# nicklashansen/tdmpc2

Measured on AMD Instinct MI355X. Metric: plan() calls/sec (H=3, 512 samples, 6 iters), higher is better.
Workload: dtype f32 (f16x2-split products: 22-bit operands, fp32 accumulate)

## Files before the change

tdmpc2_amd/csrc/fused_kernels.cuh:

```cuda
#pragma once

#include "kloop_schedule.h"

#ifdef SPLIT_TIMING
#define TIMER_FIELDS mutable unsigned long long t_acc[14] = {0, 0, 0, 0, 0, 0, 0, 0, 0, 0, 0, 0, 0, 0}; mutable unsigned long long t_last = 0, t_begin = 0;
#define TIMER_START(c) { (c).t_last = (c).t_begin = __builtin_amdgcn_s_memtime(); }
#define TIMER_MARK(c, cls) { __builtin_amdgcn_sched_barrier(0); const unsigned long long t_now = __builtin_amdgcn_s_memtime(); __builtin_amdgcn_sched_barrier(0); (c).t_acc[cls] += t_now - (c).t_last; (c).t_last = t_now; }
#ifndef SPLIT_TIMING_WAVE
#define SPLIT_TIMING_WAVE 4
#endif
#define TIMER_FLUSH(c, ptr) if ((ptr) && threadIdx.x == 64 * SPLIT_TIMING_WAVE) { for (int i_ = 0; i_ < 14; ++i_) atomicAdd((ptr) + i_, (c).t_acc[i_]); atomicAdd((ptr) + 14, (c).t_last - (c).t_begin); atomicAdd((ptr) + 15, 1ull); }
#else
#define TIMER_FIELDS
#define TIMER_START(c)
#define TIMER_MARK(c, cls)
#define TIMER_FLUSH(c, ptr)
#endif
enum { T_KLOOP = 0, T_EPI = 1, T_HEAD = 2, T_ACT = 3, T_PARK = 4, T_TILE = 5, T_EPI_PRE = 6, T_EPI_SYNC = 7, T_EPI_BIAS = 8,
       T_EPI_COMB = 9, T_EPI_MATH = 10, T_CL_WAIT = 11, T_HEAD_K = 12, T_HEAD_ST = 13 };



#ifdef KS_NO_BIAS_LDS
constexpr bool KS_BIAS_LDS = false;
#else
constexpr bool KS_BIAS_LDS = true;
#endif
#ifdef KS_NO_ZH_REGS
constexpr bool KS_ZH_REGS = false;
#else
constexpr bool KS_ZH_REGS = true;
#endif
template <int APAD, int ST = 2, int NW = 8, int AR = 0>
struct CtxT {
    static constexpr bool BIAS_LDS = false;
    static constexpr int NST = ST;
    static constexpr int NWAVES = NW;
    static constexpr int ARITH = AR;
    static constexpr int FT = 16 / NW;
    static constexpr int NTHR = 64 * NW;
    static constexpr int TROWS = 32 * ST;
    static constexpr int SH = WIDTH + APAD;
    static constexpr int RSH = 2 * SH + 8;
    static constexpr int RSF_ = AR == 0 ? RSH / 2 : WIDTH + APAD + 4;
    static constexpr int KBLK = AR == 0 ? 16 : 8;
    static constexpr int ZKB = WIDTH / KBLK;
    _Float16 *act;
    float *stats;
    float *gb;
    int tid, wave, lane;
    mutable float pg[(WIDTH + NTHR - 1) / NTHR], pb[(WIDTH + NTHR - 1) / NTHR];
    TIMER_FIELDS
    __device__ __forceinline__ float *f32() const { return reinterpret_cast<float *>(act); }
    static constexpr __device__ __forceinline__ int RSF() { return RSF_; }
};
template <int APAD, int ST, int NW, int AR>
struct CtxPhT : CtxT<APAD, ST, NW, AR> {
    static constexpr bool BIAS_LDS = KS_BIAS_LDS;
    mutable float pbias = 0.f;
};

__device__ __forceinline__ float mish_fast(float x) {
    const float e = __expf(fminf(x, 20.f));
    const float n = e * (e + 2.f);
    return x * (n * __builtin_amdgcn_rcpf(n + 2.f));
}

template <class CT>
__device__ __forceinline__ float exp_a(float x) {
    if constexpr (CT::ARITH == 1) return expf(x);
    else return __expf(x);
}
template <class CT>
__device__ __forceinline__ float mish_a(float x) {
    if constexpr (CT::ARITH == 1) {
        const float e = expf(fminf(x, 20.f));
        const float n = e * (e + 2.f);
        return x * (n / (n + 2.f));
    } else {
        return mish_fast(x);
    }
}

__device__ __forceinline__ void split4(const f32x4 y, f16x4 &hi, f16x4 &lo, const float scale = ACT_SCALE) {
#pragma unroll
    for (int e = 0; e < 4; ++e) {
        const float ys = y[e] * scale;
        const _Float16 h = (_Float16)ys;
        hi[e] = h;
        lo[e] = (_Float16)(ys - (float)h);
    }
}


constexpr int PF = 2;
template <int FT>
struct BFragT {
    f16x8 h[FT], l[FT];
};
__device__ __forceinline__ f16x8 ldw(const char *ubase, unsigned voff, int imm) {
    return *reinterpret_cast<const f16x8 *>(ubase + voff + imm);
}
#define SPLIT_MFMA(a, b, c) __builtin_amdgcn_mfma_f32_32x32x16_f16(a, b, c, 0, 0, 0)
template <int FT>
__device__ __forceinline__ void load_b(BFragT<FT> &b, const char *u0, size_t ct_stride, unsigned voff) {
#pragma unroll
    for (int cc = 0; cc < FT; ++cc) {
        b.h[cc] = ldw(u0 + cc * ct_stride, voff, 0);
        b.l[cc] = ldw(u0 + cc * ct_stride, voff, 1024);
    }
}
template <int ST, int FT>
__device__ __forceinline__ void zero_acc(f32x16 (&a)[ST][FT]) {
#pragma unroll
    for (int r = 0; r < ST; ++r)
#pragma unroll
        for (int cc = 0; cc < FT; ++cc)
#pragma unroll
            for (int e = 0; e < 16; ++e) a[r][cc][e] = 0.f;
}
template <int ST>
struct AFragT {
    f16x8 h[ST], l[ST];
};
template <class CT>
__device__ __forceinline__ void load_a(AFragT<CT::NST> &a, const _Float16 *a0p, int kk) {
#pragma unroll
    for (int st = 0; st < CT::NST; ++st) {
        a.h[st] = *reinterpret_cast<const f16x8 *>(a0p + st * 32 * CT::RSH + kk * 16);
        a.l[st] = *reinterpret_cast<const f16x8 *>(a0p + st * 32 * CT::RSH + CT::SH + kk * 16);
    }
}
template <class CT>
__device__ __forceinline__ void kloop_f32(const CT &c, const LayerS &ly, int kb0, int kb1, f32x16 (&acc)[CT::NST][CT::FT]) {
    constexpr int FT = CT::FT, NST = CT::NST;
    constexpr int PFD = 4;
    const int i = c.lane & 31, hh = c.lane >> 5;
    const float *a0p = c.f32() + i * CT::RSF() + 4 * hh + kb0 * 8;
    const char *u0 = reinterpret_cast<const char *>(ly.wp) + ((size_t)(FT * c.wave) * ly.KB + kb0) * 1024;
    const size_t cts = (size_t)ly.KB * 1024;
    unsigned voff = (unsigned)c.lane * 16u;
    asm volatile("" : "+v"(voff));
    const int nk = kb1 - kb0;
    f32x4 ring[PFD][FT];
#pragma unroll
    for (int d = 0; d < PFD; ++d) {
        const int kd = d < nk ? d : nk - 1;
#pragma unroll
        for (int cc = 0; cc < FT; ++cc) ring[d][cc] = *reinterpret_cast<const f32x4 *>(u0 + (size_t)kd * 1024 + cc * cts + voff);
    }
    f32x4 an[NST];
#pragma unroll
    for (int st = 0; st < NST; ++st) an[st] = *reinterpret_cast<const f32x4 *>(a0p + st * 32 * CT::RSF());
    __builtin_amdgcn_sched_barrier(0);
#pragma unroll 1
    for (int k = 0; k < nk; k += PFD) {
#pragma unroll
        for (int d = 0; d < PFD; ++d) {
            const int kk = k + d;
            if (kk < nk) {
                f32x4 a[NST];
                const int kx = kk + 1 < nk ? kk + 1 : kk;
#pragma unroll
                for (int st = 0; st < NST; ++st) {
                    a[st] = an[st];
                    an[st] = *reinterpret_cast<const f32x4 *>(a0p + st * 32 * CT::RSF() + kx * 8);
                }
#pragma unroll
                for (int r = 0; r < 4; ++r)
#pragma unroll
                    for (int cc = 0; cc < FT; ++cc)
#pragma unroll
                        for (int st = 0; st < NST; ++st)
                            acc[st][cc] = __builtin_amdgcn_mfma_f32_32x32x2f32(ring[d][cc][r], a[st][r], acc[st][cc], 0, 0, 0);
                const int kn = kk + PFD < nk ? kk + PFD : nk - 1;
#pragma unroll
                for (int cc = 0; cc < FT; ++cc)
                    ring[d][cc] = *reinterpret_cast<const f32x4 *>(u0 + (size_t)kn * 1024 + cc * cts + voff);
                __builtin_amdgcn_sched_barrier(0);
            }
        }
    }
}

#define A_MFMA(ACC, WF, AF) asm volatile("v_mfma_f32_32x32x16_f16 %0, %1, %2, %0" : "+v"(ACC) : "v"(WF), "v"(AF))
template <int OFF>
__device__ __forceinline__ void a_dsrd(f16x8 &dst, unsigned addr) {
    asm volatile("ds_read_b128 %0, %1 offset:%2" : "=v"(dst) : "v"(addr), "n"(OFF));
}
__device__ __forceinline__ unsigned lds_addr_of(const void *p) {
    return (unsigned)(size_t)(const __attribute__((address_space(3))) char *)(p);
}
template <class CT>
__device__ __forceinline__ void a_load_act(AFragT<CT::NST> &a, unsigned la0, unsigned la1) {
    a_dsrd<0>(a.h[0], la0);
    a_dsrd<2 * CT::SH>(a.l[0], la0);
    if constexpr (CT::NST == 2) {
        a_dsrd<0>(a.h[1], la1);
        a_dsrd<2 * CT::SH>(a.l[1], la1);
    }
}
__device__ __forceinline__ void a_load_w(BFragT<2> &b, unsigned voff, const char *s0, const char *s1) {
    asm volatile("s_nop 4\n\t"
                 "global_load_dwordx4 %0, %4, %5\n\t"
                 "global_load_dwordx4 %1, %4, %5 offset:1024\n\t"
                 "global_load_dwordx4 %2, %4, %6\n\t"
                 "global_load_dwordx4 %3, %4, %6 offset:1024"
                 : "=&v"(b.h[0]), "=&v"(b.l[0]), "=&v"(b.h[1]), "=&v"(b.l[1])
                 : "v"(voff), "s"(s0), "s"(s1));
}
template <class CT>
// ... 186 lines not shown
#pragma unroll
            for (int e = 0; e < 16; ++e) acc[r][t][e] = 0.f;
    f16x8 rh[PFT], rl[PFT];
#pragma unroll
    for (int d = 0; d < PFT; ++d) {
        const int kd = d < nk ? d : nk - 1;
        rh[d] = ldw(u + (size_t)kd * 2048, voff, 0);
        rl[d] = ldw(u + (size_t)kd * 2048, voff, 1024);
    }
    AFragT<CT::NST> an;
    load_a<CT>(an, a0p, 0);
    __builtin_amdgcn_sched_barrier(0);
    auto step = [&](const int kk, const int d, const bool steady) __attribute__((always_inline)) {
        const AFragT<CT::NST> a = an;
        load_a<CT>(an, a0p, (steady || kk + 1 < nk) ? kk + 1 : kk);
#pragma unroll
        for (int st = 0; st < CT::NST; ++st) acc[st][0] = SPLIT_MFMA(a.h[st], rh[d], acc[st][0]);
#pragma unroll
        for (int st = 0; st < CT::NST; ++st) acc[st][1] = SPLIT_MFMA(a.h[st], rl[d], acc[st][1]);
#pragma unroll
        for (int st = 0; st < CT::NST; ++st) acc[st][2] = SPLIT_MFMA(a.l[st], rh[d], acc[st][2]);
        const int kn = (steady || kk + PFT < nk) ? kk + PFT : nk - 1;
        rh[d] = ldw(u + (size_t)kn * 2048, voff, 0);
        rl[d] = ldw(u + (size_t)kn * 2048, voff, 1024);
        __builtin_amdgcn_sched_barrier(0);
    };
    int k = 0;
#pragma unroll 1
    for (; k + 2 * PFT <= nk; k += PFT) {
#pragma unroll
        for (int d = 0; d < PFT; ++d) step(k + d, d, true);
    }
#pragma unroll 1
    for (; k < nk; k += PFT) {
#pragma unroll
        for (int d = 0; d < PFT; ++d)
            if (k + d < nk) step(k + d, d, false);
    }
#pragma unroll
    for (int r = 0; r < CT::NST; ++r)
#pragma unroll
        for (int e = 0; e < 16; ++e) out[r][e] = acc[r][0][e] + (acc[r][1][e] + acc[r][2][e]);
}


template <class CT>
__device__ __forceinline__ void park(const CT &c, const f32x16 (&acc)[CT::NST][CT::FT], float *dst) {
#pragma unroll
    for (int st = 0; st < CT::NST; ++st)
#pragma unroll
        for (int ft = 0; ft < CT::FT; ++ft)
#pragma unroll
            for (int m = 0; m < 4; ++m) {
                f32x4 v;
#pragma unroll
                for (int r = 0; r < 4; ++r) v[r] = acc[st][ft][4 * m + r];
                const int idx4 = ((c.wave * CT::NST + st) * CT::FT + ft) * 4 + m;
                *reinterpret_cast<f32x4 *>(dst + ((size_t)idx4 * 64 + c.lane) * 4) = v;
            }
}
template <class CT>
__device__ __forceinline__ void unpark(const CT &c, f32x16 (&acc)[CT::NST][CT::FT], const float *src) {
#pragma unroll
    for (int st = 0; st < CT::NST; ++st)
#pragma unroll
        for (int ft = 0; ft < CT::FT; ++ft)
#pragma unroll
            for (int m = 0; m < 4; ++m) {
                const int idx4 = ((c.wave * CT::NST + st) * CT::FT + ft) * 4 + m;
                const f32x4 v = *reinterpret_cast<const f32x4 *>(src + ((size_t)idx4 * 64 + c.lane) * 4);
#pragma unroll
                for (int r = 0; r < 4; ++r) acc[st][ft][4 * m + r] = v[r];
            }
}

template <class CT>
__device__ __forceinline__ void regs_to_tile(const CT &c, const f32x16 (&y)[CT::NST][CT::FT], const float scale = ACT_SCALE) {
    const int j = c.lane & 31, hh = c.lane >> 5;
    if constexpr (CT::ARITH == 1) {
#pragma unroll
        for (int st = 0; st < CT::NST; ++st) {
            float *fp = c.f32() + (32 * st + j) * CT::RSF() + 32 * CT::FT * c.wave + 4 * hh;
#pragma unroll
            for (int ft = 0; ft < CT::FT; ++ft)
#pragma unroll
                for (int m = 0; m < 4; ++m) {
                    f32x4 v;
#pragma unroll
                    for (int r = 0; r < 4; ++r) v[r] = y[st][ft][4 * m + r];
                    *reinterpret_cast<f32x4 *>(fp + 32 * ft + 8 * m) = v;
                }
        }
        return;
    }
#pragma unroll
    for (int st = 0; st < CT::NST; ++st) {
        _Float16 *hp = c.act + (32 * st + j) * c.RSH + 32 * CT::FT * c.wave + 4 * hh;
#pragma unroll
        for (int ft = 0; ft < CT::FT; ++ft)
#pragma unroll
            for (int m = 0; m < 4; ++m) {
                f32x4 v;
#pragma unroll
                for (int r = 0; r < 4; ++r) v[r] = y[st][ft][4 * m + r];
                f16x4 hi, lo;
                split4(v, hi, lo, scale);
                *reinterpret_cast<f16x4 *>(hp + 32 * ft + 8 * m) = hi;
                *reinterpret_cast<f16x4 *>(hp + c.SH + 32 * ft + 8 * m) = lo;
            }
    }
}

struct GB {
    const float *g = nullptr, *b = nullptr, *bias = nullptr;
};
__device__ __forceinline__ GB gb_of(const LayerS &ly) { return GB{ly.g, ly.b, ly.bias}; }
__device__ __forceinline__ GB gb_of(const LayerS &ly, const float *bias) { return GB{ly.g, ly.b, bias}; }

template <class CT>
__device__ __forceinline__ void gb_prefetch(const CT &c, const float *g, const float *b) {
#pragma unroll
    for (int u = 0; u < (WIDTH + CT::NTHR - 1) / CT::NTHR; ++u) {
        const int f = c.tid + u * CT::NTHR;
        c.pg[u] = f < WIDTH ? g[f] : 0.f;
        c.pb[u] = f < WIDTH ? b[f] : 0.f;
    }
}
template <class CT>
__device__ __forceinline__ void gb_prefetch(const CT &c, const GB next) {
    gb_prefetch(c, next.g, next.b);
    if constexpr (CT::BIAS_LDS) {
        static_assert(CT::FT == 2 && CT::NTHR == WIDTH, "thread tid fetches feature tid of its own wave's 64");
        c.pbias = next.bias[c.tid];
    }
}
template <class CT>
__device__ __forceinline__ void gb_commit(const CT &c) {
    if constexpr (CT::BIAS_LDS) c.stats[c.wave * (CT::TROWS * 2) + c.lane] = c.pbias;
#pragma unroll
    for (int u = 0; u < (WIDTH + CT::NTHR - 1) / CT::NTHR; ++u) {
        const int f = c.tid + u * CT::NTHR;
        if (f < WIDTH) {
            c.gb[f] = c.pg[u];
            c.gb[WIDTH + f] = c.pb[u];
        }
    }
}
template <class CT>
__device__ __forceinline__ void epi_barrier(const CT &c) {
    __syncthreads();
    gb_commit(c);
}

enum { EPI_PRE = 1, EPI_MATH = 2, EPI_STORE = 4, EPI_ALL = 7 };
template <int ACT, class CT, bool HASBIAS = true, int PIECES = EPI_ALL>
__device__ __forceinline__ void epi_t(const CT &c, f32x16 (&acc)[CT::NST][CT::FT], float osc, float asc, const float *bias,
                                      GB next, float *zcopy) {
    constexpr int FT = CT::FT, NW = CT::NWAVES;
    constexpr float CNT = 32.f * FT;
    const int j = c.lane & 31, hh = c.lane >> 5;
    const int poff = 32 * FT * c.wave + 4 * hh;
    if constexpr (PIECES & EPI_PRE) {
    if constexpr (HASBIAS) {
#pragma unroll
        for (int ft = 0; ft < FT; ++ft) {
            f32x4 b4[4];
#pragma unroll
            for (int m = 0; m < 4; ++m) {
                if constexpr (CT::BIAS_LDS)
                    b4[m] = *reinterpret_cast<const f32x4 *>(c.stats + c.wave * (CT::TROWS * 2) + 4 * hh + 32 * ft + 8 * m);
                else b4[m] = *reinterpret_cast<const f32x4 *>(bias + poff + 32 * ft + 8 * m);
            }
#pragma unroll
            for (int m = 0; m < 4; ++m)
#pragma unroll
                for (int st = 0; st < CT::NST; ++st)
#pragma unroll
                    for (int r = 0; r < 4; ++r) acc[st][ft][4 * m + r] = fmaf(acc[st][ft][4 * m + r], osc, b4[m][r]);
        }
    }
    TIMER_MARK(c, T_EPI_BIAS)
#pragma unroll
    for (int st = 0; st < CT::NST; ++st) {
        float s = 0.f;
#pragma unroll
        for (int ft = 0; ft < FT; ++ft)
#pragma unroll
            for (int e = 0; e < 16; ++e) s += acc[st][ft][e];
        s += __shfl_xor(s, 32);
        const float mw = s * (1.0f / CNT);
        float m2 = 0.f;
#pragma unroll
        for (int ft = 0; ft < FT; ++ft)
#pragma unroll
            for (int e = 0; e < 16; ++e) {
                const float d = acc[st][ft][e] - mw;
                m2 = fmaf(d, d, m2);
            }
        m2 += __shfl_xor(m2, 32);
        if (hh == 0) {
            c.stats[(c.wave * CT::TROWS + 32 * st + j) * 2 + 0] = mw;
            c.stats[(c.wave * CT::TROWS + 32 * st + j) * 2 + 1] = m2;
        }
    }
    TIMER_MARK(c, T_EPI_PRE)
    }
    if constexpr (PIECES == EPI_ALL) {
    __syncthreads();
    TIMER_MARK(c, T_EPI_SYNC)
    }
    if constexpr (PIECES & EPI_MATH) {
    float rstd[CT::NST], shift[CT::NST];
#pragma unroll
    for (int st = 0; st < CT::NST; ++st) {
        float pm[NW], mean = 0.f, msum = 0.f;
#pragma unroll
        for (int w = 0; w < NW; ++w) {
            pm[w] = c.stats[(w * CT::TROWS + 32 * st + j) * 2 + 0];
            msum += c.stats[(w * CT::TROWS + 32 * st + j) * 2 + 1];
            mean += pm[w];
        }
        mean *= 1.0f / NW;
#pragma unroll
        for (int w = 0; w < NW; ++w) {
            const float d = pm[w] - mean;
            msum = fmaf(CNT * d, d, msum);
        }
        rstd[st] = 1.0f / sqrtf(msum * (1.0f / WIDTH) + LN_EPS);
        shift[st] = -mean * rstd[st];
    }
    TIMER_MARK(c, T_EPI_COMB)
#pragma unroll
    for (int ft = 0; ft < FT; ++ft) {
        f32x4 gq[4], bq[4];
#pragma unroll
        for (int m = 0; m < 4; ++m) {
            gq[m] = *reinterpret_cast<const f32x4 *>(c.gb + poff + 32 * ft + 8 * m);
            bq[m] = *reinterpret_cast<const f32x4 *>(c.gb + WIDTH + poff + 32 * ft + 8 * m);
        }
#pragma unroll
        for (int m = 0; m < 4; ++m) {
            const f32x4 g4 = gq[m], b4 = bq[m];
#pragma unroll
            for (int st = 0; st < CT::NST; ++st) {
                float y[4];
#pragma unroll
                for (int r = 0; r < 4; ++r) y[r] = fmaf(fmaf(acc[st][ft][4 * m + r], rstd[st], shift[st]), g4[r], b4[r]);
                if (ACT == 0) {
#pragma unroll
                    for (int r = 0; r < 4; ++r) y[r] = mish_a<CT>(y[r]);
                } else {
                    float mx = fmaxf(fmaxf(y[0], y[1]), fmaxf(y[2], y[3]));
                    mx = fmaxf(mx, __shfl_xor(mx, 32));
                    float es = 0.f;
#pragma unroll
                    for (int r = 0; r < 4; ++r) {
                        y[r] = exp_a<CT>(y[r] - mx);
                        es += y[r];
                    }
                    es += __shfl_xor(es, 32);
                    if constexpr (CT::ARITH == 1) {
#pragma unroll
                        for (int r = 0; r < 4; ++r) y[r] = y[r] / es;
                    } else {
                        const float inv = 1.0f / es;
#pragma unroll
                        for (int r = 0; r < 4; ++r) y[r] *= inv;
                    }
                }
#pragma unroll
                for (int r = 0; r < 4; ++r) acc[st][ft][4 * m + r] = y[r];
            }
        }
    }
    }
    if constexpr (PIECES & EPI_STORE) {
    regs_to_tile(c, acc, ACT == 0 ? asc : ACT_SCALE);
    TIMER_MARK(c, T_EPI_MATH)
    if (zcopy) park(c, acc, zcopy);
    }
}
template <class CT>
__device__ __forceinline__ void epi_pre(const CT &c, f32x16 (&acc)[CT::NST][CT::FT], float osc, const float *bias) {
    epi_t<0, CT, true, EPI_PRE>(c, acc, osc, 0.f, bias, GB{}, nullptr);
}
template <int ACT, class CT>
__device__ __forceinline__ void epi_math(const CT &c, f32x16 (&acc)[CT::NST][CT::FT], float asc) {
    epi_t<ACT, CT, true, EPI_MATH>(c, acc, 0.f, asc, nullptr, GB{}, nullptr);
}
template <int ACT, class CT>
__device__ __forceinline__ void epi_store(const CT &c, f32x16 (&acc)[CT::NST][CT::FT], float asc, float *zcopy) {
    epi_t<ACT, CT, true, EPI_STORE>(c, acc, 0.f, asc, nullptr, GB{}, zcopy);
}

template <class CT>
__device__ __forceinline__ void add_row_bias(const CT &c, f32x16 (&acc)[CT::NST][CT::FT], float osc, const float *const (&brow)[CT::NST]) {
    const int hh = c.lane >> 5;
    const int poff = 32 * CT::FT * c.wave + 4 * hh;
#pragma unroll
    for (int st = 0; st < CT::NST; ++st)
#pragma unroll
        for (int ft = 0; ft < CT::FT; ++ft)
#pragma unroll
            for (int m = 0; m < 4; ++m) {
                const f32x4 b4 = *reinterpret_cast<const f32x4 *>(brow[st] + poff + 32 * ft + 8 * m);
#pragma unroll
                for (int r = 0; r < 4; ++r) acc[st][ft][4 * m + r] = fmaf(acc[st][ft][4 * m + r], osc, b4[r]);
            }
}

template <class CT>
__device__ __forceinline__ void store_tile_s(const CT &c, const f32x16 &acc, float osc, const float *bias, int ct, int rt) {
    float *f = c.f32();
    constexpr int RSF = CT::RSF();
    const int j = c.lane & 31, hh = c.lane >> 5;
    const int col = ct * 32 + j;
    const float bv = bias[col];
#pragma unroll
    for (int reg = 0; reg < 16; ++reg) {
        const int row = rt * 32 + (reg & 3) + 8 * (reg >> 2) + 4 * hh;
        f[row * RSF + col] = fmaf(acc[reg], osc, bv);
    }
}

template <class CT>
__device__ __forceinline__ float twohot_rows_s(const CT &c, const float *bins, int num_bins) {
    const int part = c.tid & 7;
    const bool live = (c.tid >> 3) < CT::TROWS;
    const int row = live ? c.tid >> 3 : 0;
    const float *rp = c.f32() + row * c.RSF();
    if (num_bins <= 1) {
        const float x1 = rp[0];
        return num_bins == 0 ? x1 : symexp_f(x1);
    }
    float v[16];
    float m = -INFINITY;
#pragma unroll
    for (int q = 0; q < 16; ++q) {
        const int jj = part + 8 * q;
        v[q] = (jj < num_bins) ? rp[jj] : -INFINITY;
        m = fmaxf(m, v[q]);
    }
    m = group_max<8>(m);
    float es = 0.f, x = 0.f;
#pragma unroll
    for (int q = 0; q < 16; ++q) {
        const int jj = part + 8 * q;
        const float ev = (jj < num_bins) ? expf(v[q] - m) : 0.f;
        es += ev;
        x = fmaf(ev, (jj < num_bins) ? bins[jj] : 0.f, x);
    }
    es = group_sum<8>(es);
    x = group_sum<8>(x);
    return symexp_f(x / es);
}

template <int ACT, class CT>
__device__ __forceinline__ void layer_full_s(const CT &c, const LayerS &ly, const float *bias, int kb0, int kb1,
                                             GB next, float *zcopy = nullptr) {
    f32x16 acc[CT::NST][CT::FT];
    zero_acc(acc);
    if (next.g) gb_prefetch(c, next);
    kloop_s(c, ly, kb0, kb1, acc);
    TIMER_MARK(c, T_KLOOP)
    epi_t<ACT>(c, acc, *ly.oscale, *ly.ascale, bias, next, zcopy);
    epi_barrier(c);
    TIMER_MARK(c, T_EPI)
}
template <int ACT, class CT>
__device__ __forceinline__ void layer_held_s(const CT &c, const LayerS &ly, const float *bias, int kb0, int kb1, GB next,
                                             f32x16 (&acc)[CT::NST][CT::FT]) {
    zero_acc(acc);
    if (next.g) gb_prefetch(c, next);
    kloop_s(c, ly, kb0, kb1, acc);
    TIMER_MARK(c, T_KLOOP)
    epi_t<ACT>(c, acc, *ly.oscale, *ly.ascale, bias, next, nullptr);
    epi_barrier(c);
    TIMER_MARK(c, T_EPI)
}

template <class CT>
__device__ __forceinline__ void head_logits_s(const CT &c, const LayerS &ly) {
    f32x16 acc[CT::NST];
    const float osc = *ly.oscale;
    const int ct = c.wave;
    if (ct < ly.CT) kloop_tile_s(c, ly, ct, 0, CT::ZKB, acc);
    __syncthreads();
    TIMER_MARK(c, T_HEAD_K)
    if (ct < ly.CT) {
#pragma unroll
        for (int rt = 0; rt < CT::NST; ++rt) store_tile_s(c, acc[rt], osc, ly.bias, ct, rt);
    }
    __syncthreads();
    TIMER_MARK(c, T_HEAD_ST)
}

template <class CT>
__device__ __forceinline__ float head_twohot_s(const CT &c, const LayerS &ly, const float *bins, int num_bins) {
    head_logits_s(c, ly);
    const float r = twohot_rows_s(c, bins, num_bins);
    __syncthreads();
    return r;
}

template <class CT>
__device__ __forceinline__ void put_action(const CT &c, int row, int a, float v) {
    if constexpr (CT::ARITH == 1) {
        c.f32()[row * CT::RSF() + WIDTH + a] = v;
        return;
    }
    const float vs = v * ACT_SCALE;
    const _Float16 h = (_Float16)vs;
    _Float16 *rp = c.act + row * c.RSH + WIDTH + a;
    rp[0] = h;
    rp[c.SH] = (_Float16)(vs - (float)h);
}

template <class CT, typename EpsFn>
__device__ __forceinline__ void head_pi_rows_s(const CT &c, int A, int Apad, float lsmin, float lsdif, const float *mask_wg, EpsFn eps,
                                               float *gdst, int nvalid, float *tsc, const float *mask_tab = nullptr,
                                               const int *row_task = nullptr, int put_rows = CT::TROWS, bool agent_store = false);

template <class CT, typename EpsFn>
__device__ __forceinline__ void head_pi_s(const CT &c, const LayerS &ly, int A, int Apad, float lsmin, float lsdif,
                                          const float *mask_wg, EpsFn eps, float *gdst, int nvalid, float *tsc,
                                          const float *mask_tab = nullptr, const int *row_task = nullptr) {
    head_logits_s(c, ly);
    head_pi_rows_s(c, A, Apad, lsmin, lsdif, mask_wg, eps, gdst, nvalid, tsc, mask_tab, row_task, CT::TROWS, false);
}

// ... 244 lines not shown
                    float r = z[u];
                    if (p.sample_eps)
                        r = p.sample_eps[(size_t)e * p.sample_eps_estride +
                                         (unsigned)(((size_t)t * (p.N - p.P) + (n - p.P)) * p.A + a)];
                    v[u] = sample_action(sm_mean[t * p.A + a], sm_std[t * p.A + a], r);
                }
                if (mask && !p.given_actions) v[u] *= mask[a];
                if (!p.given_actions) ag[(size_t)n * p.A + a] = v[u];
            }
            put_action(c, row, a, v[u]);
        }
    }
}

#define DUMP_TILE(...) do { if constexpr (TRACE) dump_tile_s(__VA_ARGS__); } while (0)
template <int APAD, int ST, int NW, int AR, int EP, int TR = 0>
__global__ __launch_bounds__(64 * NW, 2) void ks_rollout(RolloutParams p) {
    constexpr bool TRACE = TR || EP;
    extern __shared__ __attribute__((aligned(16))) float smem[];
    __shared__ int s_is_last;
    const int e = blockIdx.x / p.tiles, tile = p.tile_off + blockIdx.x % p.tiles;
    const int tid = threadIdx.x;
    typedef CtxPhT<APAD, ST, NW, AR> CT;
    constexpr int TROWS = CT::TROWS, NTHR = CT::NTHR, FT = CT::FT;
    constexpr int ZKB16 = CT::ZKB;
    constexpr bool ZH_REGS = !EP && KS_ZH_REGS;
    CT c{{reinterpret_cast<_Float16 *>(smem), smem + TROWS * CT::RSF(), smem + TROWS * CT::RSF() + 1024, tid,
          __builtin_amdgcn_readfirstlane(tid >> 6), tid & 63}};
    float *sm_mean = smem + TROWS * CT::RSF() + 2048;
    float *sm_std = sm_mean + p.H * p.A;
    const int row0 = tile * TROWS;
    const float *mask = p.act_mask ? p.act_mask + (size_t)e * p.A : nullptr;
    const float *disc = p.disc_pow + (size_t)e * (p.H + 1);
    const int KBA = ZKB16 + p.Apad / CT::KBLK;
    float *zs = p.zscratch + (size_t)blockIdx.x * TROWS * WIDTH;
    const int NSLOT = 5 * p.H + 7;
    const bool live = (tid >> 3) < TROWS;
    float *tsc = nullptr;
    if constexpr (TRACE) tsc = p.trace_scalars && live ? p.trace_scalars + ((size_t)e * p.N + row0 + (tid >> 3)) * (p.H + 2 + p.A) : nullptr;

    for (int idx = tid; idx < p.H * p.A; idx += NTHR) {
        sm_mean[idx] = p.mean[(size_t)e * p.H * p.A + idx];
        sm_std[idx] = p.std[(size_t)e * p.H * p.A + idx];
    }
    int q0, q1;
    if (p.qidx) {
        q0 = p.qidx[(size_t)e * p.qidx_estride + 0];
        q1 = p.qidx[(size_t)e * p.qidx_estride + 1];
    } else {
        const uint4 r = rng_raw(p.seed, p.call, SITE_QIDX, p.iter, e, 0);
        q0 = (int)(r.x % (unsigned)p.nq);
        q1 = (int)(r.y % (unsigned)(p.nq - 1));
        if (q1 >= q0) ++q1;
    }
    const float *b_rew = p.multitask ? p.beff + ((size_t)e * p.nnets + BE_REW) * WIDTH : p.rew.l[0].bias;
    const float *b_dyn = p.multitask ? p.beff + ((size_t)e * p.nnets + BE_DYN) * WIDTH : p.dyn.l[0].bias;
    const float *b_pi = p.multitask ? p.beff + ((size_t)e * p.nnets + BE_PI) * WIDTH : p.pi.l[0].bias;
    const float *b_q0 = p.multitask ? p.beff + ((size_t)e * p.nnets + BE_Q0 + q0) * WIDTH : p.q[q0].l[0].bias;
    const float *b_q1 = p.multitask ? p.beff + ((size_t)e * p.nnets + BE_Q0 + q1) * WIDTH : p.q[q1].l[0].bias;
    const float *c_rew = p.cvec + ((size_t)e * 2 + 0) * WIDTH, *c_dyn = p.cvec + ((size_t)e * 2 + 1) * WIDTH;
    gb_prefetch(c, gb_of(p.rew.l[0], c_rew));
    epi_barrier(c);

    float G = 0.f;
    float termv = 0.f;
    TIMER_START(c)
    for (int t = 0; t < p.H; ++t) {
        sample_actions(c, p, e, row0, mask, sm_mean, sm_std, t);
        __syncthreads();
        TIMER_MARK(c, T_ACT)
        const bool term_step = EP && t > 0;
        f32x16 accd[ST][FT];
        {
            f32x16 acc[ST][FT];
            gb_prefetch(c, gb_of(p.rew.l[1]));
            first_layers_s(c, p.dyn.l[0], p.rew.l[0], t == 0 ? ZKB16 : 0, KBA, accd, acc);
            TIMER_MARK(c, T_KLOOP)
            if constexpr (EP) {
                if (term_step) {
                    park(c, accd, zs);
                    zero_acc(accd);
                    kloop_s(c, p.term.l[0], 0, ZKB16, accd);
                }
            }
            epi_t<0>(c, acc, *p.rew.l[0].oscale, *p.rew.l[0].ascale, t == 0 ? c_rew : b_rew, gb_of(p.rew.l[1]), nullptr);
        }
        epi_barrier(c);
        TIMER_MARK(c, T_EPI)
        DUMP_TILE(c, p.trace_tiles, NSLOT, 5 * t + 0, p.rew.l[0].ascale);
        layer_full_s<0>(c, p.rew.l[1], p.rew.l[1].bias, 0, ZKB16,
                        term_step ? gb_of(p.term.l[0]) : gb_of(p.dyn.l[0], t == 0 ? c_dyn : b_dyn));
        DUMP_TILE(c, p.trace_tiles, NSLOT, 5 * t + 1, p.rew.l[1].ascale);
        if (term_step) gb_prefetch(c, gb_of(p.term.l[1]));
        else gb_prefetch(c, gb_of(p.dyn.l[1]));
        const float r = head_twohot_s(c, p.rew.l[2], p.bins, p.num_bins);
        TIMER_MARK(c, T_HEAD)
        if (tsc && (tid & 7) == 0) tsc[t] = r;
        if constexpr (EP) {
            if (term_step) {
                epi_t<0>(c, accd, *p.term.l[0].oscale, *p.term.l[0].ascale, p.term.l[0].bias, gb_of(p.term.l[1]), nullptr);
                epi_barrier(c);
                layer_full_s<0>(c, p.term.l[1], p.term.l[1].bias, 0, ZKB16, gb_of(p.dyn.l[0], b_dyn));
                gb_prefetch(c, gb_of(p.dyn.l[1]));
                termv = fminf(termv + head_term_s(c, p.term.l[2]), 1.f);
                unpark(c, accd, zs);
            }
        }
        G += disc[t] * (1.f - termv) * r;
        epi_t<0>(c, accd, *p.dyn.l[0].oscale, *p.dyn.l[0].ascale, t == 0 ? c_dyn : b_dyn, gb_of(p.dyn.l[1]), nullptr);
        epi_barrier(c);
        TIMER_MARK(c, T_EPI)
        DUMP_TILE(c, p.trace_tiles, NSLOT, 5 * t + 2, p.dyn.l[0].ascale);
        layer_full_s<0>(c, p.dyn.l[1], p.dyn.l[1].bias, 0, ZKB16, gb_of(p.dyn.l[2]));
        DUMP_TILE(c, p.trace_tiles, NSLOT, 5 * t + 3, p.dyn.l[1].ascale);
        if constexpr (ZH_REGS) {
            if (t == p.H - 1) break;
            layer_full_s<1>(c, p.dyn.l[2], p.dyn.l[2].bias, 0, ZKB16, gb_of(p.rew.l[0], b_rew), nullptr);
        } else {
            layer_full_s<1>(c, p.dyn.l[2], p.dyn.l[2].bias, 0, ZKB16,
                            t == p.H - 1 ? gb_of(p.pi.l[0], b_pi) : gb_of(p.rew.l[0], b_rew), t == p.H - 1 ? zs : nullptr);
        }
        DUMP_TILE(c, p.trace_tiles, NSLOT, 5 * t + 4);
    }
    f32x16 acch[ST][FT];
    if constexpr (ZH_REGS) {
        layer_held_s<1>(c, p.dyn.l[2], p.dyn.l[2].bias, 0, ZKB16, gb_of(p.pi.l[0], b_pi), acch);
        DUMP_TILE(c, p.trace_tiles, NSLOT, 5 * (p.H - 1) + 4);
    }
    if constexpr (EP) {
        zero_acc(acch);
        kloop_s(c, p.term.l[0], 0, ZKB16, acch);
    }
    layer_full_s<0>(c, p.pi.l[0], b_pi, 0, ZKB16, gb_of(p.pi.l[1]));
    DUMP_TILE(c, p.trace_tiles, NSLOT, 5 * p.H + 0, p.pi.l[0].ascale);
    layer_full_s<0>(c, p.pi.l[1], p.pi.l[1].bias, 0, ZKB16, EP ? gb_of(p.term.l[0]) : gb_of(p.q[q0].l[0], b_q0));
    DUMP_TILE(c, p.trace_tiles, NSLOT, 5 * p.H + 1, p.pi.l[1].ascale);
    if constexpr (EP) gb_prefetch(c, gb_of(p.term.l[1]));
    {
        auto eps = [&](int row, int a) -> float {
            const unsigned ridx = (unsigned)((size_t)(row0 + row) * p.A + a);
            if (p.pi_eps) return p.pi_eps[(size_t)e * p.pi_eps_estride + ridx];
            return rng_normal(p.seed, p.call, SITE_PI, p.iter, e, ridx);
        };
        head_pi_s(c, p.pi.l[2], p.A, p.Apad, p.log_std_min, p.log_std_dif, mask, eps, nullptr, 0,
                  tsc ? tsc + p.H + 2 : nullptr);
    }
    TIMER_MARK(c, T_HEAD)
    if constexpr (EP) {
        epi_t<0>(c, acch, *p.term.l[0].oscale, *p.term.l[0].ascale, p.term.l[0].bias, gb_of(p.term.l[1]), nullptr);
        epi_barrier(c);
        layer_full_s<0>(c, p.term.l[1], p.term.l[1].bias, 0, ZKB16, gb_of(p.q[q0].l[0], b_q0));
        termv = fminf(termv + head_term_s(c, p.term.l[2]), 1.f);
    }
    if constexpr (ZH_REGS) regs_to_tile(c, acch);
    else tile_from_global_s(c, zs);
    __syncthreads();
    TIMER_MARK(c, T_TILE)
    DUMP_TILE(c, p.trace_tiles, NSLOT, 5 * p.H + 2);
    {
        f32x16 acc[ST][FT];
        gb_prefetch(c, gb_of(p.q[q0].l[1]));
        first_layers_s(c, p.q[q1].l[0], p.q[q0].l[0], 0, KBA, acch, acc);
        TIMER_MARK(c, T_KLOOP)
        epi_t<0>(c, acc, *p.q[q0].l[0].oscale, *p.q[q0].l[0].ascale, b_q0, gb_of(p.q[q0].l[1]), nullptr);
    }
    epi_barrier(c);
    TIMER_MARK(c, T_EPI)
    DUMP_TILE(c, p.trace_tiles, NSLOT, 5 * p.H + 3, p.q[q0].l[0].ascale);
    layer_full_s<0>(c, p.q[q0].l[1], p.q[q0].l[1].bias, 0, ZKB16, gb_of(p.q[q1].l[0], b_q1));
    DUMP_TILE(c, p.trace_tiles, NSLOT, 5 * p.H + 4, p.q[q0].l[1].ascale);
    gb_prefetch(c, gb_of(p.q[q1].l[1]));
    const float qa = head_twohot_s(c, p.q[q0].l[2], p.bins, p.num_bins);
    TIMER_MARK(c, T_HEAD)
    epi_t<0>(c, acch, *p.q[q1].l[0].oscale, *p.q[q1].l[0].ascale, b_q1, gb_of(p.q[q1].l[1]), nullptr);
    epi_barrier(c);
    TIMER_MARK(c, T_EPI)
    DUMP_TILE(c, p.trace_tiles, NSLOT, 5 * p.H + 5, p.q[q1].l[0].ascale);
    layer_full_s<0>(c, p.q[q1].l[1], p.q[q1].l[1].bias, 0, ZKB16, GB{});
    DUMP_TILE(c, p.trace_tiles, NSLOT, 5 * p.H + 6, p.q[q1].l[1].ascale);
    const float qb = head_twohot_s(c, p.q[q1].l[2], p.bins, p.num_bins);
    TIMER_MARK(c, T_HEAD)
    TIMER_FLUSH(c, p.timing)
    if (tsc && (tid & 7) == 0) {
        tsc[p.H] = qa;
        tsc[p.H + 1] = qb;
    }
    const float val = G + disc[p.H] * (1.f - termv) * ((qa + qb) / 2.f);
    if (!p.fold_refit) {
        if ((tid & 7) == 0 && live) p.value[(size_t)e * p.N + row0 + (tid >> 3)] = val;
        return;
    }
    if ((tid & 7) == 0 && live)
        __hip_atomic_store(p.value + (size_t)e * p.N + row0 + (tid >> 3), val, __ATOMIC_RELAXED, __HIP_MEMORY_SCOPE_AGENT);
    asm volatile("s_waitcnt vmcnt(0)" ::: "memory");
    __builtin_amdgcn_fence(__ATOMIC_RELEASE, "workgroup");
    __syncthreads();
    if (tid == 0) {
        const unsigned old = __hip_atomic_fetch_add(p.ticket + e, 1u, __ATOMIC_RELAXED, __HIP_MEMORY_SCOPE_AGENT);
        const int last = old == (unsigned)(p.tiles - 1);
        if (last) __hip_atomic_store(p.ticket + e, 0u, __ATOMIC_RELAXED, __HIP_MEMORY_SCOPE_AGENT);
        s_is_last = last;
    }
    __syncthreads();
    if (!s_is_last) return;
    refit_plan(p.rf, e, smem, tid, NTHR);
}

template <int APAD, int AR>
__global__ __launch_bounds__(NTHREADS, 2) void ks_value(ValueParams p) {
    extern __shared__ __attribute__((aligned(16))) float smem[];
    const int tid = threadIdx.x;
    typedef CtxT<APAD, 2, 8, AR> CT;
    constexpr int TROWS = CT::TROWS, ZKB16 = CT::ZKB;
    CT c{reinterpret_cast<_Float16 *>(smem), smem + TROWS * CT::RSF(), smem + TROWS * CT::RSF() + 1024, tid,
         __builtin_amdgcn_readfirstlane(tid >> 6), tid & 63};
    int *s_task = reinterpret_cast<int *>(smem + TROWS * CT::RSF() + 2048);
    const int row0 = blockIdx.x * TROWS;
    const int nvalid = min(TROWS, p.rows - row0);
    const float *zsrc = p.z + (size_t)row0 * WIDTH;
    const int KBA = ZKB16 + p.Apad / CT::KBLK;
    int q0, q1;
    if (p.qidx) {
        q0 = p.qidx[0];
        q1 = p.qidx[1];
    } else {
        const uint4 r = rng_raw(p.seed, p.call, SITE_QIDX, 0, 0, 0);
        q0 = (int)(r.x % (unsigned)p.nq);
        q1 = (int)(r.y % (unsigned)(p.nq - 1));
        if (q1 >= q0) ++q1;
    }
    if (p.task_ids && tid < TROWS) s_task[tid] = tid < nvalid ? p.task_ids[row0 + tid] : 0;
    tile_from_rows_s(c, zsrc, nvalid);
    gb_prefetch(c, p.pi.l[0].g, p.pi.l[0].b);
    epi_barrier(c);
    const int j = c.lane & 31;
    auto first_layer = [&](const LayerS &ly, int slot, int kb1, GB next) {
        if (!p.task_ids) {
            layer_full_s<0>(c, ly, ly.bias, 0, kb1, next);
            return;
        }
        const float *brow[CT::NST];
#pragma unroll
        for (int st = 0; st < CT::NST; ++st) brow[st] = p.beff_tab + ((size_t)s_task[32 * st + j] * p.nnets + slot) * WIDTH;
        f32x16 acc[CT::NST][CT::FT];
        zero_acc(acc);
        if (next.g) gb_prefetch(c, next.g, next.b);
        kloop_s(c, ly, 0, kb1, acc);
        add_row_bias(c, acc, *ly.oscale, brow);
        epi_t<0, CT, false>(c, acc, 1.f, *ly.ascale, nullptr, next, nullptr);
        epi_barrier(c);
    };
    first_layer(p.pi.l[0], BE_PI, ZKB16, gb_of(p.pi.l[1]));
    layer_full_s<0>(c, p.pi.l[1], p.pi.l[1].bias, 0, ZKB16, gb_of(p.q[q0].l[0]));
    {
        auto eps = [&](int row, int a) -> float {
            const unsigned ridx = (unsigned)((size_t)(row0 + row) * p.A + a);
            if (p.pi_eps) return row < nvalid ? p.pi_eps[ridx] : 0.f;
            return rng_normal(p.seed, p.call, SITE_PI, 0, 0, ridx);
        };
        head_pi_s(c, p.pi.l[2], p.A, p.Apad, p.log_std_min, p.log_std_dif, nullptr, eps,
                  p.action ? p.action + (size_t)row0 * p.A : nullptr, nvalid, nullptr, p.task_ids ? p.mask_tab : nullptr, s_task);
    }
    tile_from_rows_s(c, zsrc, nvalid);
    __syncthreads();
    first_layer(p.q[q0].l[0], BE_Q0 + q0, KBA, gb_of(p.q[q0].l[1]));
    layer_full_s<0>(c, p.q[q0].l[1], p.q[q0].l[1].bias, 0, ZKB16, gb_of(p.q[q1].l[0]));
    const float qa = head_twohot_s(c, p.q[q0].l[2], p.bins, p.num_bins);
    tile_from_rows_s(c, zsrc, nvalid);
    __syncthreads();
    first_layer(p.q[q1].l[0], BE_Q0 + q1, KBA, gb_of(p.q[q1].l[1]));
    layer_full_s<0>(c, p.q[q1].l[1], p.q[q1].l[1].bias, 0, ZKB16, GB{});
    const float qb = head_twohot_s(c, p.q[q1].l[2], p.bins, p.num_bins);
    const int row = tid >> 3;
    if ((tid & 7) == 0 && row < nvalid) {
        float v = p.reduce_min ? fminf(qa, qb) : (qa + qb) / 2.f;
        if (p.reward) {
            const float disc = p.disc_tab ? p.disc_tab[s_task[row]] : p.discount;
            v = p.reward[row0 + row] + disc * (1.f - p.terminated[row0 + row]) * v;
        }
        p.out[row0 + row] = v;
    }
}
```

Measured before the change: 10240.

## Interleave LayerNorm epilogue math into independent packed chains with scheduling fences

Adds chain-structured versions of the epilogue statistics, combine, and normalize/activation/f16-split-store code. They interleave the row tiles and pack element pairs into f32x2 operations, with sched_barrier fences placed to keep several independent dependency chains in flight. The goal is to hide ALU latency in the serial reductions and the mish/softmax sequence, and to fuse the store into the math loop. In exchange the compiler loses freedom to schedule around the fences, and register pressure may rise. An asm barrier on acch is also added before regs_to_tile.

```diff
diff --git a/tdmpc2_amd/csrc/fused_kernels.cuh b/tdmpc2_amd/csrc/fused_kernels.cuh
--- a/tdmpc2_amd/csrc/fused_kernels.cuh
+++ b/tdmpc2_amd/csrc/fused_kernels.cuh
@@ -21,6 +21,16 @@
 
 
 
+#ifdef KS_NO_STAT_CHAINS
+constexpr bool KS_STAT_CHAINS = false;
+#else
+constexpr bool KS_STAT_CHAINS = true;
+#endif
+#ifdef KS_NO_EPI_CHAINS
+constexpr bool KS_EPI_CHAINS = false;
+#else
+constexpr bool KS_EPI_CHAINS = true;
+#endif
 #ifdef KS_NO_BIAS_LDS
 constexpr bool KS_BIAS_LDS = false;
 #else
@@ -37,6 +47,7 @@
     static constexpr int NST = ST;
     static constexpr int NWAVES = NW;
     static constexpr int ARITH = AR;
+    static constexpr bool STAT_CHAINS = false, EPI_CHAINS = false;
     static constexpr int FT = 16 / NW;
     static constexpr int NTHR = 64 * NW;
     static constexpr int TROWS = 32 * ST;
@@ -57,6 +68,8 @@
 template <int APAD, int ST, int NW, int AR>
 struct CtxPhT : CtxT<APAD, ST, NW, AR> {
     static constexpr bool BIAS_LDS = KS_BIAS_LDS;
+    static constexpr bool STAT_CHAINS = KS_STAT_CHAINS && AR == 0;
+    static constexpr bool EPI_CHAINS = KS_EPI_CHAINS && AR == 0;
     mutable float pbias = 0.f;
 };
 
@@ -549,6 +562,231 @@
     gb_commit(c);
 }
 
+template <class CT>
+__device__ __forceinline__ void stats_chains(const CT &c, const f32x16 (&acc)[CT::NST][CT::FT]) {
+    constexpr int FT = CT::FT, NST = CT::NST;
+    constexpr float CNT = 32.f * FT;
+    const int j = c.lane & 31, hh = c.lane >> 5;
+    float s[NST], sx[NST], mw[NST], m2[NST];
+#pragma unroll
+    for (int st = 0; st < NST; ++st) s[st] = 0.f;
+#pragma unroll
+    for (int ft = 0; ft < FT; ++ft)
+#pragma unroll
+        for (int e = 0; e < 16; ++e) {
+#pragma unroll
+            for (int st = 0; st < NST; ++st) s[st] += acc[st][ft][e];
+            if ((e & 3) == 3) __builtin_amdgcn_sched_barrier(0);
+        }
+#pragma unroll
+    for (int st = 0; st < NST; ++st) sx[st] = __shfl_xor(s[st], 32);
+#pragma unroll
+    for (int st = 0; st < NST; ++st) {
+        s[st] += sx[st];
+        mw[st] = s[st] * (1.0f / CNT);
+        m2[st] = 0.f;
+    }
+#pragma unroll
+    for (int ft = 0; ft < FT; ++ft)
+#pragma unroll
+        for (int m = 0; m < 4; ++m) {
+            float d[NST][4];
+#pragma unroll
+            for (int r = 0; r < 4; ++r)
+#pragma unroll
+                for (int st = 0; st < NST; ++st) d[st][r] = acc[st][ft][4 * m + r] - mw[st];
+            __builtin_amdgcn_sched_barrier(0);
+#pragma unroll
+            for (int r = 0; r < 4; ++r)
+#pragma unroll
+                for (int st = 0; st < NST; ++st) m2[st] = fmaf(d[st][r], d[st][r], m2[st]);
+        }
+#pragma unroll
+    for (int st = 0; st < NST; ++st) sx[st] = __shfl_xor(m2[st], 32);
+#pragma unroll
+    for (int st = 0; st < NST; ++st) {
+        m2[st] += sx[st];
+        if (hh == 0) {
+            c.stats[(c.wave * CT::TROWS + 32 * st + j) * 2 + 0] = mw[st];
+            c.stats[(c.wave * CT::TROWS + 32 * st + j) * 2 + 1] = m2[st];
+        }
+    }
+}
+template <class CT>
+__device__ __forceinline__ void combine_chains(const CT &c, float (&rstd)[CT::NST], float (&shift)[CT::NST]) {
+    constexpr int NW = CT::NWAVES, NST = CT::NST;
+    constexpr float CNT = 32.f * CT::FT;
+    const int j = c.lane & 31;
+    float pm[NST][NW], mean[NST], msum[NST], sd[NST];
+#pragma unroll
+    for (int st = 0; st < NST; ++st) mean[st] = msum[st] = 0.f;
+#pragma unroll
+    for (int w = 0; w < NW; ++w)
+#pragma unroll
+        for (int st = 0; st < NST; ++st) {
+            pm[st][w] = c.stats[(w * CT::TROWS + 32 * st + j) * 2 + 0];
+            msum[st] += c.stats[(w * CT::TROWS + 32 * st + j) * 2 + 1];
+            mean[st] += pm[st][w];
+        }
+#pragma unroll
+    for (int st = 0; st < NST; ++st) mean[st] *= 1.0f / NW;
+#pragma unroll
+    for (int w = 0; w < NW; ++w)
+#pragma unroll
+        for (int st = 0; st < NST; ++st) {
+            const float d = pm[st][w] - mean[st];
+            msum[st] = fmaf(CNT * d, d, msum[st]);
+        }
+#pragma unroll
+    for (int st = 0; st < NST; ++st) sd[st] = sqrtf(msum[st] * (1.0f / WIDTH) + LN_EPS);
+#pragma unroll
+    for (int st = 0; st < NST; ++st) rstd[st] = 1.0f / sd[st];
+#pragma unroll
+    for (int st = 0; st < NST; ++st) shift[st] = -mean[st] * rstd[st];
+}
+typedef float f32x2 __attribute__((ext_vector_type(2)));
+typedef _Float16 f16x2 __attribute__((ext_vector_type(2)));
+template <class V>
+__device__ __forceinline__ void chain_fence(V (&)[4]) {
+    __builtin_amdgcn_sched_barrier(0);
+}
+#define CHAIN_PAIRS _Pragma("unroll") for (int p = 0; p < 4; ++p)
+template <int ACT, bool MATH, bool STORE, class CT>
+__device__ __forceinline__ void epi_chains(const CT &c, f32x16 (&acc)[CT::NST][CT::FT], const float (&rstd)[CT::NST],
+                                           const float (&shift)[CT::NST], const float scale) {
+#pragma clang fp contract(off)
+    static_assert(CT::ARITH == 0 && (CT::NST == 1 || CT::NST == 2), "f16x2 split, one or two row tiles");
+    constexpr int FT = CT::FT, NST = CT::NST, MG = 2 / NST, NG = FT * 4 / MG;
+    constexpr float LOG2E = 0x1.715476p+0f;
+    const int j = c.lane & 31, hh = c.lane >> 5;
+    const int poff = 32 * FT * c.wave + 4 * hh;
+    f32x4 gq[MG], bq[MG], gn[MG], bn[MG];
+    if constexpr (MATH) {
+#pragma unroll
+        for (int mi = 0; mi < MG; ++mi) {
+            gq[mi] = *reinterpret_cast<const f32x4 *>(c.gb + poff + 8 * mi);
+            bq[mi] = *reinterpret_cast<const f32x4 *>(c.gb + WIDTH + poff + 8 * mi);
+        }
+    }
+#pragma unroll
+    for (int g = 0; g < NG; ++g) {
+        const int ft = (g * MG) >> 2, m0 = (g * MG) & 3;
+#define CH_ST(p) (NST == 2 ? (p) >> 1 : 0)
+#define CH_MI(p) (NST == 2 ? 0 : (p) >> 1)
+#define CH_REG(p) (4 * (m0 + CH_MI(p)) + 2 * ((p) & 1))
+        f32x2 y[4];
+        if constexpr (MATH) {
+            if (g + 1 < NG) {
+                const int fn = ((g + 1) * MG) >> 2, mn = ((g + 1) * MG) & 3;
+#pragma unroll
+                for (int mi = 0; mi < MG; ++mi) {
+                    gn[mi] = *reinterpret_cast<const f32x4 *>(c.gb + poff + 32 * fn + 8 * (mn + mi));
+                    bn[mi] = *reinterpret_cast<const f32x4 *>(c.gb + WIDTH + poff + 32 * fn + 8 * (mn + mi));
+                }
+            }
+            CHAIN_PAIRS {
+                const f32x2 a2 = {acc[CH_ST(p)][ft][CH_REG(p)], acc[CH_ST(p)][ft][CH_REG(p) + 1]};
+                const f32x2 r2 = {rstd[CH_ST(p)], rstd[CH_ST(p)]}, s2 = {shift[CH_ST(p)], shift[CH_ST(p)]};
+                y[p] = __builtin_elementwise_fma(a2, r2, s2);
+            }
+            chain_fence(y);
+            CHAIN_PAIRS {
+                const f32x4 g4 = gq[CH_MI(p)], b4 = bq[CH_MI(p)];
+                const f32x2 g2 = {g4[2 * (p & 1)], g4[2 * (p & 1) + 1]}, b2 = {b4[2 * (p & 1)], b4[2 * (p & 1) + 1]};
+                y[p] = __builtin_elementwise_fma(y[p], g2, b2);
+            }
+            chain_fence(y);
+            if constexpr (ACT == 0) {
+                f32x2 a[4], e[4], n[4];
+                CHAIN_PAIRS a[p] = f32x2{fminf(y[p].x, 20.f), fminf(y[p].y, 20.f)};
+                chain_fence(a);
+                CHAIN_PAIRS a[p] = a[p] * LOG2E;
+                chain_fence(a);
+                CHAIN_PAIRS e[p] = f32x2{__builtin_amdgcn_exp2f(a[p].x), __builtin_amdgcn_exp2f(a[p].y)};
+                chain_fence(e);
+                CHAIN_PAIRS a[p] = e[p] + 2.f;
+                chain_fence(a);
+                CHAIN_PAIRS n[p] = e[p] * a[p];
+                chain_fence(n);
+                CHAIN_PAIRS a[p] = n[p] + 2.f;
+                chain_fence(a);
+                CHAIN_PAIRS a[p] = f32x2{__builtin_amdgcn_rcpf(a[p].x), __builtin_amdgcn_rcpf(a[p].y)};
+                chain_fence(a);
+                CHAIN_PAIRS n[p] = n[p] * a[p];
+                chain_fence(n);
+                CHAIN_PAIRS y[p] = y[p] * n[p];
+                chain_fence(y);
+            } else {
+                float mx[2], px[2], es[2], inv[2];
+#pragma unroll
+                for (int q = 0; q < 2; ++q) mx[q] = fmaxf(fmaxf(y[2 * q].x, y[2 * q].y), fmaxf(y[2 * q + 1].x, y[2 * q + 1].y));
+#pragma unroll
+                for (int q = 0; q < 2; ++q) px[q] = __shfl_xor(mx[q], 32);
+#pragma unroll
+                for (int q = 0; q < 2; ++q) mx[q] = fmaxf(mx[q], px[q]);
+                CHAIN_PAIRS y[p] = y[p] - mx[p >> 1];
+                chain_fence(y);
+                CHAIN_PAIRS y[p] = y[p] * LOG2E;
+                chain_fence(y);
+                CHAIN_PAIRS y[p] = f32x2{__builtin_amdgcn_exp2f(y[p].x), __builtin_amdgcn_exp2f(y[p].y)};
+                chain_fence(y);
+#pragma unroll
+                for (int q = 0; q < 2; ++q) es[q] = 0.f;
+#pragma unroll
+                for (int r = 0; r < 4; ++r)
+#pragma unroll
+                    for (int q = 0; q < 2; ++q) es[q] += y[2 * q + (r >> 1)][r & 1];
+#pragma unroll
+                for (int q = 0; q < 2; ++q) px[q] = __shfl_xor(es[q], 32);
+#pragma unroll
+                for (int q = 0; q < 2; ++q) es[q] += px[q];
+#pragma unroll
+                for (int q = 0; q < 2; ++q) inv[q] = 1.0f / es[q];
+                CHAIN_PAIRS y[p] = y[p] * inv[p >> 1];
+                chain_fence(y);
+            }
+            CHAIN_PAIRS {
+                acc[CH_ST(p)][ft][CH_REG(p)] = y[p].x;
+                acc[CH_ST(p)][ft][CH_REG(p) + 1] = y[p].y;
+            }
+            if (g + 1 < NG) {
+#pragma unroll
+                for (int mi = 0; mi < MG; ++mi) {
+                    gq[mi] = gn[mi];
+                    bq[mi] = bn[mi];
+                }
+            }
+        } else {
+            CHAIN_PAIRS y[p] = f32x2{acc[CH_ST(p)][ft][CH_REG(p)], acc[CH_ST(p)][ft][CH_REG(p) + 1]};
+        }
+        if constexpr (STORE) {
+            f32x2 ys[4];
+            f16x2 h[4], l[4];
+            CHAIN_PAIRS ys[p] = y[p] * scale;
+            chain_fence(ys);
+            CHAIN_PAIRS h[p] = __builtin_convertvector(ys[p], f16x2);
+            chain_fence(h);
+            CHAIN_PAIRS ys[p] = __builtin_convertvector(h[p], f32x2);
+            chain_fence(ys);
+            CHAIN_PAIRS ys[p] = __builtin_elementwise_fma(y[p], f32x2{scale, scale}, -ys[p]);
+            chain_fence(ys);
+            CHAIN_PAIRS l[p] = __builtin_convertvector(ys[p], f16x2);
+#pragma unroll
+            for (int q = 0; q < 2; ++q) {
+                const f16x4 hi = {h[2 * q].x, h[2 * q].y, h[2 * q + 1].x, h[2 * q + 1].y};
+                const f16x4 lo = {l[2 * q].x, l[2 * q].y, l[2 * q + 1].x, l[2 * q + 1].y};
+                _Float16 *hp = c.act + (32 * CH_ST(2 * q) + j) * c.RSH + poff + 32 * ft + 8 * (m0 + CH_MI(2 * q));
+                *reinterpret_cast<f16x4 *>(hp) = hi;
+                *reinterpret_cast<f16x4 *>(hp + c.SH) = lo;
+            }
+        }
+#undef CH_ST
+#undef CH_MI
+#undef CH_REG
+    }
+}
+#undef CHAIN_PAIRS
+
 enum { EPI_PRE = 1, EPI_MATH = 2, EPI_STORE = 4, EPI_ALL = 7 };
 template <int ACT, class CT, bool HASBIAS = true, int PIECES = EPI_ALL>
 __device__ __forceinline__ void epi_t(const CT &c, f32x16 (&acc)[CT::NST][CT::FT], float osc, float asc, const float *bias,
@@ -577,6 +815,8 @@
         }
     }
     TIMER_MARK(c, T_EPI_BIAS)
+    if constexpr (CT::STAT_CHAINS) stats_chains(c, acc);
+    else
 #pragma unroll
     for (int st = 0; st < CT::NST; ++st) {
         float s = 0.f;
@@ -608,6 +848,8 @@
     }
     if constexpr (PIECES & EPI_MATH) {
     float rstd[CT::NST], shift[CT::NST];
+    if constexpr (CT::STAT_CHAINS) combine_chains(c, rstd, shift);
+    else
 #pragma unroll
     for (int st = 0; st < CT::NST; ++st) {
         float pm[NW], mean = 0.f, msum = 0.f;
@@ -630,6 +872,9 @@
 #pragma unroll
     for (int ft = 0; ft < FT; ++ft) {
         f32x4 gq[4], bq[4];
+        if constexpr (CT::EPI_CHAINS) {
+            if (ft == 0) epi_chains<ACT, true, PIECES == EPI_ALL>(c, acc, rstd, shift, ACT == 0 ? asc : ACT_SCALE);
+        } else {
 #pragma unroll
         for (int m = 0; m < 4; ++m) {
             gq[m] = *reinterpret_cast<const f32x4 *>(c.gb + poff + 32 * ft + 8 * m);
@@ -669,10 +914,16 @@
                 for (int r = 0; r < 4; ++r) acc[st][ft][4 * m + r] = y[r];
             }
         }
+        }
     }
     }
     if constexpr (PIECES & EPI_STORE) {
-    regs_to_tile(c, acc, ACT == 0 ? asc : ACT_SCALE);
+    if constexpr (CT::EPI_CHAINS) {
+        if constexpr (PIECES != EPI_ALL) {
+            const float none[CT::NST] = {};
+            epi_chains<ACT, false, true>(c, acc, none, none, ACT == 0 ? asc : ACT_SCALE);
+        }
+    } else regs_to_tile(c, acc, ACT == 0 ? asc : ACT_SCALE);
     TIMER_MARK(c, T_EPI_MATH)
     if (zcopy) park(c, acc, zcopy);
     }
@@ -1223,7 +1474,15 @@
         layer_full_s<0>(c, p.term.l[1], p.term.l[1].bias, 0, ZKB16, gb_of(p.q[q0].l[0], b_q0));
         termv = fminf(termv + head_term_s(c, p.term.l[2]), 1.f);
     }
-    if constexpr (ZH_REGS) regs_to_tile(c, acch);
+    if constexpr (ZH_REGS) {
+        if constexpr (CT::EPI_CHAINS) {
+#pragma unroll
+            for (int st = 0; st < ST; ++st)
+#pragma unroll
+                for (int ft = 0; ft < FT; ++ft) asm volatile("" : "+v"(acch[st][ft]));
+        }
+        regs_to_tile(c, acch);
+    }
     else tile_from_global_s(c, zs);
     __syncthreads();
     TIMER_MARK(c, T_TILE)
```

Measured after the change: 10280, median of 6. No clear change (+0.4%).
